# yixuan/ADMM

Measured on AMD Instinct MI355X. Metric: ADMM iterations/sec, Lasso tall n=100000 p=10000 (100-lambda warm-started path), higher is better.
Workload: dtype f32; 1 GPU; admm_lasso tall path (BASELINE configs[1]); n=100000, p=10000, nlambda=100, standardize=True, intercept=True, parallelism=single GPU, step=one cold-started warm-chained lambda path

## Files before the change

### admm_amd/csrc/symv_kernels.h

```cpp
#pragma once
#include "admm_internal.h"
#include "device_utils.h"
#include "symv_pack.h"
#include <hip/hip_ext.h>
#include <climits>
#include <type_traits>

namespace admm {

constexpr int kSyRB = 256;
constexpr int kSyCB = 128;
constexpr int kSyCBMax = 256;
static_assert(kSyCBMax == 256, "SYMV_SCHED's widths are checked against 256 where the option is parsed (options.hip)");
constexpr int kSyThreads = 256;

struct SymvSched {
    int width_big = kSyCB, width_small = kSyCB;
    int rb_split = 0;
    __host__ __device__ int width(int rb) const { return rb >= rb_split ? width_big : width_small; }
    __host__ __device__ int nseg(int rb, int p32) const {
        const int cols = min((rb + 1) * kSyRB, p32), w = width(rb);
        return (cols + w - 1) / w;
    }
};
constexpr int kSySumLanes = 8;

struct SymvArgs {
    const float* A; long long lda; int p;
    const float* v0; const float* v1;
    float* dot0; float* dot1;
    float* axp0; float* axp1;
    long long ldo;
    const int4* tiles;
    const int* skip;
    const unsigned long long* verdict;
    unsigned long long discard;
    unsigned long long* early;
#ifdef ADMM_HIP_PROBE
    long long* probe; int probe_idx;
#endif
};

constexpr int kSyVerdictReplicas = 64;
constexpr int kSyVerdictStride = 16;
struct SymvVerdict {
    const unsigned long long* words = nullptr;
    unsigned long long discard = 0;
    unsigned long long* early = nullptr;
    bool mid = false;
};

template <typename T>
__device__ __forceinline__ T butterfly8(const T (&v)[8], int lane) {
    T a4[4], a2[2];
    {
        const int b = (lane >> 5) & 1;
#pragma unroll
        for (int k = 0; k < 4; ++k) {
            const T keep = b ? v[k + 4] : v[k], send = b ? v[k] : v[k + 4];
            a4[k] = keep + __shfl_xor(send, 32, 64);
        }
    }
    {
        const int b = (lane >> 4) & 1;
#pragma unroll
        for (int k = 0; k < 2; ++k) {
            const T keep = b ? a4[k + 2] : a4[k], send = b ? a4[k] : a4[k + 2];
            a2[k] = keep + __shfl_xor(send, 16, 64);
        }
    }
    const int b = (lane >> 3) & 1;
    const T keep = b ? a2[1] : a2[0], send = b ? a2[0] : a2[1];
    T r = keep + __shfl_xor(send, 8, 64);
    r += __shfl_xor(r, 4, 64);
    r += __shfl_xor(r, 2, 64);
    r += __shfl_xor(r, 1, 64);
    return r;
}

struct SymvPlainVec {
    __device__ __forceinline__ float4 load4(const float* p) const { return *reinterpret_cast<const float4*>(p); }
    __device__ __forceinline__ float load1(const float* p) const { return *p; }
};
struct SymvBypassVec {
    __device__ __forceinline__ float4 load4(const float* p) const {
        const unsigned long long lo = __hip_atomic_load(reinterpret_cast<const unsigned long long*>(p), __ATOMIC_RELAXED, __HIP_MEMORY_SCOPE_AGENT);
        const unsigned long long hi = __hip_atomic_load(reinterpret_cast<const unsigned long long*>(p) + 1, __ATOMIC_RELAXED, __HIP_MEMORY_SCOPE_AGENT);
        return make_float4(__uint_as_float((unsigned)lo), __uint_as_float((unsigned)(lo >> 32)), __uint_as_float((unsigned)hi), __uint_as_float((unsigned)(hi >> 32)));
    }
    __device__ __forceinline__ float load1(const float* p) const {
        return __uint_as_float(__hip_atomic_load(reinterpret_cast<const unsigned int*>(p), __ATOMIC_RELAXED, __HIP_MEMORY_SCOPE_AGENT));
    }
};
struct SymvNoWait { __device__ __forceinline__ void operator()() const {} };

template <bool PRE, typename Wait, typename VecLoad, bool NT = false, bool MID = false>
__device__ __forceinline__ void symv2_tile(const SymvArgs& a, const int4 t, Wait wait, VecLoad vl,
                                           float4 (*red)[kSyThreads], float (*sdot)[kSyCBMax]) {
    const int rb = t.x, seg = t.w;
    const int cw = t.z >> 2;
    const int lane = threadIdx.x & 63, wid = threadIdx.x >> 6;
    const int row = rb * kSyRB + lane * 4;
    const int col0 = t.y + wid * cw;
    const int p4 = (a.p + 3) & ~3;
    const bool active = row < p4;
    const bool has = col0 < a.p;
    const float* base = a.A + (size_t)col0 * a.lda + row;
    float4 av[8];
    if (PRE) {
#pragma unroll
        for (int k = 0; k < 8; ++k) {
            av[k] = make_float4(0.f, 0.f, 0.f, 0.f);
            if (has && active && col0 + k < a.p) av[k] = *reinterpret_cast<const float4*>(base + (size_t)k * a.lda);
        }
        wait();
    }
    float4 aU = make_float4(0.f, 0.f, 0.f, 0.f), aW = aU;

    if (has) {
        const float4 uI = active ? vl.load4(a.v0 + row) : make_float4(0.f, 0.f, 0.f, 0.f);
        const float4 wI = active ? vl.load4(a.v1 + row) : make_float4(0.f, 0.f, 0.f, 0.f);
        const int cj = col0 + lane;
        const float uj = (lane < cw && cj < a.p) ? vl.load1(a.v0 + cj) : 0.f;
        const float wj = (lane < cw && cj < a.p) ? vl.load1(a.v1 + cj) : 0.f;
        const bool diag = col0 + (cw - 1) >= rb * kSyRB;
        const int nq = cw >> 3;
        const int last = active ? min(a.p - 1, diag ? row + 3 : INT_MAX) : -1;
        const unsigned long long* vword = a.verdict + (size_t)(blockIdx.x & (kSyVerdictReplicas - 1)) * kSyVerdictStride;
#pragma unroll 1
        for (int q = 0; q < nq; ++q) {
            unsigned long long vq = 0;
            if constexpr (MID) vq = __hip_atomic_load(vword, __ATOMIC_RELAXED, __HIP_MEMORY_SCOPE_AGENT);
            if (!PRE || q > 0) {
#pragma unroll
                for (int k = 0; k < 8; ++k) {
                    const int col = col0 + q * 8 + k;
                    av[k] = make_float4(0.f, 0.f, 0.f, 0.f);
                    if constexpr (NT) { if (col <= last) av[k] = load16_nt<float4>(base + (size_t)(q * 8 + k) * a.lda); }
                    else { if (col <= last) av[k] = *reinterpret_cast<const float4*>(base + (size_t)(q * 8 + k) * a.lda); }
                }
            }
            if constexpr (MID) {
                const unsigned lo = __builtin_amdgcn_readfirstlane((unsigned)vq), hi = __builtin_amdgcn_readfirstlane((unsigned)(vq >> 32));
                if ((((unsigned long long)hi << 32) | lo) == a.discard) break;
            }
            float dU[8], dW[8];
#pragma unroll
            for (int k = 0; k < 8; ++k) {
                const int col = col0 + q * 8 + k;
                float4 v = av[k];
                float4 ax = v;
                if (diag) {
                    if (row + 0 < col) v.x = 0.f;
                    if (row + 1 < col) v.y = 0.f;
                    if (row + 2 < col) v.z = 0.f;
                    if (row + 3 < col) v.w = 0.f;
                    ax = v;
                    if (row + 0 == col) ax.x = 0.f;
                    if (row + 1 == col) ax.y = 0.f;
                    if (row + 2 == col) ax.z = 0.f;
                    if (row + 3 == col) ax.w = 0.f;
                }
                dU[k] = fmaf(v.x, uI.x, fmaf(v.y, uI.y, fmaf(v.z, uI.z, v.w * uI.w)));
                dW[k] = fmaf(v.x, wI.x, fmaf(v.y, wI.y, fmaf(v.z, wI.z, v.w * wI.w)));
                const float ujc = __int_as_float(__builtin_amdgcn_readlane(__float_as_int(uj), (q * 8 + k) & 63));
                const float wjc = __int_as_float(__builtin_amdgcn_readlane(__float_as_int(wj), (q * 8 + k) & 63));
                aU.x = fmaf(ax.x, ujc, aU.x); aU.y = fmaf(ax.y, ujc, aU.y); aU.z = fmaf(ax.z, ujc, aU.z); aU.w = fmaf(ax.w, ujc, aU.w);
                aW.x = fmaf(ax.x, wjc, aW.x); aW.y = fmaf(ax.y, wjc, aW.y); aW.z = fmaf(ax.z, wjc, aW.z); aW.w = fmaf(ax.w, wjc, aW.w);
            }
            const float du = butterfly8(dU, lane);
            const float dw = butterfly8(dW, lane);
            if ((lane & 7) == 0) {
                sdot[0][wid * cw + q * 8 + (lane >> 3)] = du;
                sdot[1][wid * cw + q * 8 + (lane >> 3)] = dw;
            }
        }
    } else {
        for (int c = lane; c < cw; c += 64) { sdot[0][wid * cw + c] = 0.f; sdot[1][wid * cw + c] = 0.f; }
    }
    red[0][threadIdx.x] = aU;
    red[1][threadIdx.x] = aW;
    __syncthreads();
    if (wid < 2) {
        float4 s = red[wid][lane];
#pragma unroll
        for (int ww = 1; ww < 4; ++ww) {
            const float4 o = red[wid][ww * 64 + lane];
            s.x += o.x; s.y += o.y; s.z += o.z; s.w += o.w;
        }
        float* dst = (wid == 0 ? a.axp0 : a.axp1) + (size_t)seg * a.ldo + row;
        *reinterpret_cast<float4*>(dst) = s;
    } else {
        float* dst = (wid == 2 ? a.dot0 : a.dot1) + (size_t)rb * a.ldo + t.y;
        for (int c = lane * 4; c < t.z; c += 256) *reinterpret_cast<float4*>(dst + c) = *reinterpret_cast<const float4*>(&sdot[wid - 2][c]);
    }
}

struct SymvNoExtra { __device__ void operator()() const {} };

template <typename Extra, bool NT = false, bool MID = false>
__global__ void __launch_bounds__(kSyThreads, 4)
symv2_lower_kernel(SymvArgs a, Extra extra) {
    if (blockIdx.x == 0) { extra(); return; }
    const int4 t = a.tiles[blockIdx.x - 1];
    const unsigned long long vw = __hip_atomic_load(a.verdict + (size_t)(blockIdx.x & (kSyVerdictReplicas - 1)) * kSyVerdictStride,
                                                    __ATOMIC_RELAXED, __HIP_MEMORY_SCOPE_AGENT);
    const int done = *a.skip;
    if (done != 0) return;
    if (vw == a.discard) {
        if (threadIdx.x == 0) atomicAdd(a.early, 1ull);
        return;
    }
    __shared__ float4 red[2][kSyThreads];
    __shared__ __attribute__((aligned(16))) float sdot[2][kSyCBMax];
#ifdef ADMM_HIP_PROBE
    const long long pt0 = wall_clock64();
#endif
    symv2_tile<false, SymvNoWait, SymvPlainVec, NT, MID>(a, t, SymvNoWait(), SymvPlainVec(), red, sdot);
#ifdef ADMM_HIP_PROBE
    if (a.probe != nullptr && threadIdx.x == 0) {
        const int nt = (int)gridDim.x - 1, t = (int)blockIdx.x - 1;
        const int which = t == 0 ? 0 : (t == nt / 2 ? 1 : (t == nt - 1 ? 2 : (t == (3 * nt) / 4 ? 3 : -1)));
        if (which >= 0) {
            long long* d = a.probe + ((size_t)(a.probe_idx & 4095) * 4 + 3) * 8 + which * 2;
            d[0] = pt0; d[1] = wall_clock64();
        }
    }
#endif
}

constexpr int kSyGateLeave = -1;
constexpr int kSyEarlySlots = kSyVerdictReplicas;
constexpr int kSyGateScratch = 6 * (kSyThreads / 64);
struct SymvForcedGate {
    struct Req {};
    int answer;
    __device__ __forceinline__ Req request() const { return Req(); }
    __device__ __forceinline__ int decide(const Req&, double*) const { return answer; }
};
#ifndef ADMM_HIP_SYMV1_WGS
#define ADMM_HIP_SYMV1_WGS 4
#endif
#ifndef ADMM_HIP_SYMV1_PRE
#define ADMM_HIP_SYMV1_PRE 8
#endif

struct SymvTileGeom { int row, col0, last, lane, wid, nqw; };

struct SymvDenseSrc {
    struct Desc {};
    __device__ __forceinline__ Desc describe(int) const { return Desc(); }
    template <bool NT>
    struct Chunk {
        const float* base; long long lda; int col0, last;
        float4 av[8];
        __device__ __forceinline__ Chunk(const SymvDenseSrc&, const Desc&, const SymvArgs& a, const SymvTileGeom& g)
            : base(a.A + (size_t)g.col0 * a.lda + g.row), lda(a.lda), col0(g.col0), last(g.last) {}
        template <int K0, int K1>
        __device__ __forceinline__ void request(int q) {
#pragma unroll
            for (int k = K0; k < K1; ++k) {
                const int col = col0 + q * 8 + k;
                av[k] = make_float4(0.f, 0.f, 0.f, 0.f);
                if constexpr (NT) { if (col <= last) av[k] = load16_nt<float4>(base + (size_t)(q * 8 + k) * lda); }
                else { if (col <= last) av[k] = *reinterpret_cast<const float4*>(base + (size_t)(q * 8 + k) * lda); }
            }
        }
        __device__ __forceinline__ void get(int, float4 (&out)[8]) const {
#pragma unroll
            for (int k = 0; k < 8; ++k) out[k] = av[k];
        }
    };
};

struct SymvPackedSrc {
    const unsigned* stream;
    const int4* ptile;
    const uint2* esc;
    int esc_cap;
    using Desc = int4;
    __device__ __forceinline__ Desc describe(int tile) const { return ptile[tile]; }
    template <bool NT>
    struct Chunk {
        const unsigned* mine;
        const uint2* esc; int nesc, ebase, col0, last, lane, chunk0;
        uint4 pc[kSpPieces]; unsigned signs;
        __device__ __forceinline__ Chunk(const SymvPackedSrc& s, const Desc& d, const SymvArgs&, const SymvTileGeom& g)
            : mine(s.stream + ((size_t)d.x + (size_t)(g.wid * g.nqw)) * kSpChunkDwords + g.lane * 4), esc(s.esc + (size_t)(blockIdx.x - 1) * s.esc_cap),
              nesc(d.z), ebase(d.y), col0(g.col0), last(g.last), lane(g.lane), chunk0(g.wid * g.nqw) {}
        template <int K0, int K1>
        __device__ __forceinline__ void request(int q) {
            if constexpr (K0 == 0 && K1 > 0) {
                const unsigned* c = mine + (size_t)q * kSpChunkDwords;
                pc[0] = make_uint4(0xEEEEEEEEu, 0xEEEEEEEEu, 0xEEEEEEEEu, 0xEEEEEEEEu);
#pragma unroll
                for (int i = 1; i < kSpPieces; ++i) pc[i] = make_uint4(0u, 0u, 0u, 0u);
                signs = 0u;
                if (col0 + q * 8 <= last) {
                    if constexpr (NT) {
#pragma unroll
                        for (int i = 0; i < kSpPieces; ++i) pc[i] = load16_nt<uint4>(c + i * 256);
                        signs = __builtin_nontemporal_load(c + 4 * kSpPieces * 64 - 3 * lane);
                    } else {
#pragma unroll
                        for (int i = 0; i < kSpPieces; ++i) pc[i] = *reinterpret_cast<const uint4*>(c + i * 256);
                        signs = c[4 * kSpPieces * 64 - 3 * lane];
                    }
                }
            }
        }
        __device__ __forceinline__ void get(int q, float4 (&out)[8]) const {
            unsigned rec[kSpRecDwords], bits[kSpEntries];
#pragma unroll
            for (int i = 0; i < kSpPieces; ++i) { rec[4 * i] = pc[i].x; rec[4 * i + 1] = pc[i].y; rec[4 * i + 2] = pc[i].z; rec[4 * i + 3] = pc[i].w; }
            rec[4 * kSpPieces] = signs;
#if ADMM_HIP_SYMV_PACK_DEC == 2
#pragma unroll
            for (int e = 0; e < kSpEntries; ++e) bits[e] = rec[e < kSpRecDwords ? e : e - 4] ^ (unsigned)ebase;
#else
            sp_record_decode(rec, ebase, bits);
#endif
#pragma unroll
            for (int k = 0; k < 8; ++k)
                out[k] = make_float4(__uint_as_float(bits[4 * k]), __uint_as_float(bits[4 * k + 1]), __uint_as_float(bits[4 * k + 2]), __uint_as_float(bits[4 * k + 3]));
            if (nesc > 0) {
                const unsigned me = ((unsigned)(chunk0 + q) << 6) | (unsigned)lane;
                for (int i = 0; i < nesc; ++i) {
                    const uint2 en = esc[i];
                    const bool hit = (en.x >> 5) == me;
                    const unsigned e = en.x & 31u;
                    const float val = __uint_as_float(en.y);
#pragma unroll
                    for (int k = 0; k < 8; ++k) {
                        if (hit && e == 4u * k + 0u) out[k].x = val;
                        if (hit && e == 4u * k + 1u) out[k].y = val;
                        if (hit && e == 4u * k + 2u) out[k].z = val;
                        if (hit && e == 4u * k + 3u) out[k].w = val;
                    }
                }
            }
        }
    };
};

template <typename Src, typename Gate, bool NT, int PRE>
__device__ __forceinline__ void symv1_tile(const SymvArgs& a, const Src& src, const Gate& gate, float4* red, float* sdot, double* gate_lds) {
    const int4 t = a.tiles[blockIdx.x - 1];
    const int done = *a.skip;
    const typename Gate::Req greq = gate.request();
    const typename Src::Desc sd = src.describe(blockIdx.x - 1);
    if (done != 0) return;
    const int rb = t.x, seg = t.w;
    const int cw = t.z >> 2;
    const int lane = threadIdx.x & 63, wid = threadIdx.x >> 6;
    const int row = rb * kSyRB + lane * 4;
    const int col0 = t.y + wid * cw;
    const int p4 = (a.p + 3) & ~3;
    const bool active = row < p4;
    const bool has = col0 < a.p;
    const bool diag = col0 + (cw - 1) >= rb * kSyRB;
    const int nq = has ? cw >> 3 : 0;
    const int last = active ? min(a.p - 1, diag ? row + 3 : INT_MAX) : -1;
    const SymvTileGeom geom = {row, col0, last, lane, wid, cw >> 3};
    typename Src::template Chunk<NT> ch(src, sd, a, geom);
    static_assert(PRE >= 0 && PRE <= 8, "columns of the first chunk requested ahead of the gate");
    if constexpr (PRE > 0) { if (nq > 0) ch.template request<0, PRE>(0); }
    const int g = gate.decide(greq, gate_lds);
    if (g == kSyGateLeave) {
        if (threadIdx.x == 0) atomicAdd(a.early + (size_t)(blockIdx.x & (kSyEarlySlots - 1)) * kSyVerdictStride, 1ull);
        return;
    }
#ifdef ADMM_HIP_PROBE
    const long long pt0 = wall_clock64();
#endif
    const float* v = g != 0 ? a.v1 : a.v0;
    float4 aU = make_float4(0.f, 0.f, 0.f, 0.f);
    if (has) {
        const float4 uI = active ? *reinterpret_cast<const float4*>(v + row) : make_float4(0.f, 0.f, 0.f, 0.f);
        const int cj = col0 + lane;
        const float uj = (lane < cw && cj < a.p) ? v[cj] : 0.f;
        const auto consume = [&](int q) {
            float4 av[8];
            ch.get(q, av);
            float dU[8];
#pragma unroll
            for (int k = 0; k < 8; ++k) {
                const int col = col0 + q * 8 + k;
                float4 m = av[k];
                float4 ax = m;
                if (diag) {
                    if (row + 0 < col) m.x = 0.f;
                    if (row + 1 < col) m.y = 0.f;
                    if (row + 2 < col) m.z = 0.f;
                    if (row + 3 < col) m.w = 0.f;
                    ax = m;
                    if (row + 0 == col) ax.x = 0.f;
                    if (row + 1 == col) ax.y = 0.f;
                    if (row + 2 == col) ax.z = 0.f;
                    if (row + 3 == col) ax.w = 0.f;
                }
                dU[k] = fmaf(m.x, uI.x, fmaf(m.y, uI.y, fmaf(m.z, uI.z, m.w * uI.w)));
                const float ujc = __int_as_float(__builtin_amdgcn_readlane(__float_as_int(uj), (q * 8 + k) & 63));
                aU.x = fmaf(ax.x, ujc, aU.x); aU.y = fmaf(ax.y, ujc, aU.y); aU.z = fmaf(ax.z, ujc, aU.z); aU.w = fmaf(ax.w, ujc, aU.w);
            }
            const float du = butterfly8(dU, lane);
            if ((lane & 7) == 0) sdot[wid * cw + q * 8 + (lane >> 3)] = du;
        };
        if constexpr (PRE > 0) { ch.template request<PRE, 8>(0); consume(0); }
#pragma unroll 1
        for (int q = PRE > 0 ? 1 : 0; q < nq; ++q) {
            ch.template request<0, 8>(q);
            consume(q);
        }
    } else {
        for (int c = lane; c < cw; c += 64) sdot[wid * cw + c] = 0.f;
    }
    red[threadIdx.x] = aU;
    __syncthreads();
    if (wid == 0) {
        float4 s = red[lane];
#pragma unroll
        for (int ww = 1; ww < 4; ++ww) {
            const float4 o = red[ww * 64 + lane];
            s.x += o.x; s.y += o.y; s.z += o.z; s.w += o.w;
        }
        *reinterpret_cast<float4*>(a.axp0 + (size_t)seg * a.ldo + row) = s;
    } else if (wid == 1) {
        float* dst = a.dot0 + (size_t)rb * a.ldo + t.y;
        for (int c = lane * 4; c < t.z; c += 256) *reinterpret_cast<float4*>(dst + c) = *reinterpret_cast<const float4*>(&sdot[c]);
    }
#ifdef ADMM_HIP_PROBE
    if (a.probe != nullptr && threadIdx.x == 0) {
        const int nt = (int)gridDim.x - 1, ti = (int)blockIdx.x - 1;
        const int which = ti == 0 ? 0 : (ti == nt / 2 ? 1 : (ti == nt - 1 ? 2 : (ti == (3 * nt) / 4 ? 3 : -1)));
        if (which >= 0) {
            long long* d = a.probe + ((size_t)(a.probe_idx & 4095) * 4 + 3) * 8 + which * 2;
            d[0] = pt0; d[1] = wall_clock64();
        }
    }
#endif
}

template <typename Gate, typename Extra, bool NT = false, int PRE = ADMM_HIP_SYMV1_PRE>
__global__ void __launch_bounds__(kSyThreads, ADMM_HIP_SYMV1_WGS)
symv1_lower_kernel(SymvArgs a, Gate gate, Extra extra) {
    if (blockIdx.x == 0) { extra(); return; }
    __shared__ float4 red[kSyThreads];
    __shared__ __attribute__((aligned(16))) float sdot[kSyCBMax];
    __shared__ double gate_lds[kSyGateScratch];
    symv1_tile<SymvDenseSrc, Gate, NT, PRE>(a, SymvDenseSrc(), gate, red, sdot, gate_lds);
}

template <typename Gate, typename Extra, bool NT = false, int PRE = ADMM_HIP_SYMV1_PRE>
__global__ void __launch_bounds__(kSyThreads, ADMM_HIP_SYMV1_WGS)
symv1_packed_kernel(SymvArgs a, SymvPackedSrc src, Gate gate, Extra extra) {
    if (blockIdx.x == 0) { extra(); return; }
    __shared__ float4 red[kSyThreads];
    __shared__ __attribute__((aligned(16))) float sdot[kSyCBMax];
    __shared__ double gate_lds[kSyGateScratch];
    symv1_tile<SymvPackedSrc, Gate, NT, PRE>(a, src, gate, red, sdot, gate_lds);
}

struct SymvPackArgs {
    const float* A; long long lda; int p;
    const int4* tiles;
    int4* ptile;
    unsigned* stream;
    uint2* esc; int esc_cap;
    unsigned long long* totals;
};
static __global__ void __launch_bounds__(kSyThreads)
symv_pack_kernel(SymvPackArgs a) {
    __shared__ int s_base;
    __shared__ unsigned s_cnt;
    const int4 t = a.tiles[blockIdx.x];
    const int rb = t.x, cw = t.z >> 2, nqw = cw >> 3;
    const int lane = threadIdx.x & 63, wid = threadIdx.x >> 6;
    const int row = rb * kSyRB + lane * 4;
    const int col0 = t.y + wid * cw;
    const int p4 = (a.p + 3) & ~3;
    const bool active = row < p4;
    if (threadIdx.x == 0) { s_base = 0; s_cnt = 0u; }
    __syncthreads();
    const float* base = a.A + (size_t)col0 * a.lda + row;
    const auto column = [&](int j, unsigned (&b)[4]) {
        const int col = col0 + j;
        b[0] = b[1] = b[2] = b[3] = 0u;
        if (active && col < a.p && row + 3 >= col) {
            const float4 m = *reinterpret_cast<const float4*>(base + (size_t)j * a.lda);
            if (row + 0 >= col) b[0] = __float_as_uint(m.x);
            if (row + 1 >= col) b[1] = __float_as_uint(m.y);
            if (row + 2 >= col) b[2] = __float_as_uint(m.z);
            b[3] = __float_as_uint(m.w);
        }
    };
    int mx = 0;
    for (int j = 0; j < cw; ++j) {
        unsigned b[4];
        column(j, b);
#pragma unroll
        for (int c = 0; c < 4; ++c) if (sp_counts(b[c])) mx = max(mx, sp_exp7(b[c]));
    }
    atomicMax(&s_base, mx);
    __syncthreads();
    const int ebase = s_base;
    const size_t first = (size_t)a.ptile[blockIdx.x].x;
    for (int q = 0; q < nqw; ++q) {
        unsigned bits[kSpEntries], rec[kSpRecDwords];
#pragma unroll
        for (int k = 0; k < 8; ++k) {
            unsigned b[4];
            column(q * 8 + k, b);
            bits[4 * k] = b[0]; bits[4 * k + 1] = b[1]; bits[4 * k + 2] = b[2]; bits[4 * k + 3] = b[3];
        }
        const unsigned em = sp_record_encode(bits, ebase, rec);
        unsigned* c = a.stream + (first + (size_t)(wid * nqw + q)) * kSpChunkDwords;
#pragma unroll
        for (int i = 0; i < kSpPieces; ++i)
            *reinterpret_cast<uint4*>(c + (i * 64 + lane) * 4) = make_uint4(rec[4 * i], rec[4 * i + 1], rec[4 * i + 2], rec[4 * i + 3]);
        c[4 * kSpPieces * 64 + lane] = rec[4 * kSpPieces];
        if (em != 0u) {
#pragma unroll
            for (int e = 0; e < kSpEntries; ++e) {
                if ((em >> e) & 1u) {
                    const unsigned slot = atomicAdd(&s_cnt, 1u);
                    if (slot < (unsigned)a.esc_cap)
                        a.esc[(size_t)blockIdx.x * a.esc_cap + slot] = make_uint2(((unsigned)(wid * nqw + q) << 11) | ((unsigned)lane << 5) | (unsigned)e, bits[e]);
                }
            }
        }
    }
    __syncthreads();
    if (threadIdx.x == 0) {
        const unsigned n = s_cnt;
        int4 d = a.ptile[blockIdx.x];
        d.y = ebase; d.z = (int)min(n, (unsigned)a.esc_cap); d.w = (int)n;
        a.ptile[blockIdx.x] = d;
        if (n != 0u) atomicAdd(a.totals, (unsigned long long)n);
        if (n > (unsigned)a.esc_cap) atomicAdd(a.totals + 1, 1ull);
    }
}

struct SymvNArgs {
    const float* A; long long lda; int p;
    const float* v; long long vstride;
    float* dot; long long dot_stride;
    float* axp; long long axp_stride;
    int nvec;
    long long ldo;
    const int4* tiles;
    const int* skip;
};
constexpr int kSyNR[] = {2, 4, 8, 12};
constexpr int kSyNRCount = (int)(sizeof(kSyNR) / sizeof(kSyNR[0]));

template <int NR, bool DIAG>
__device__ __forceinline__ void symvn_chunk(float4 (&av)[8], const float4 (&vI)[NR], const float (&vj)[NR], float4 (&acc)[NR],
                                            int row, int colq, int q, int lane, float (*sdot)[kSyCBMax], int sbase) {
    float4 ax[DIAG ? 8 : 1];
    if (DIAG) {
#pragma unroll
        for (int k = 0; k < 8; ++k) {
            const int col = colq + k;
            float4 v = av[k];
            if (row + 0 < col) v.x = 0.f;
            if (row + 1 < col) v.y = 0.f;
            if (row + 2 < col) v.z = 0.f;
            if (row + 3 < col) v.w = 0.f;
            av[k] = v;
            if (row + 0 == col) v.x = 0.f;
            if (row + 1 == col) v.y = 0.f;
            if (row + 2 == col) v.z = 0.f;
            if (row + 3 == col) v.w = 0.f;
            ax[DIAG ? k : 0] = v;
        }
    }
#pragma unroll
    for (int r = 0; r < NR; ++r) {
        float d[8];
        const float4 xi = vI[r];
        float4 s = acc[r];
#pragma unroll
        for (int k = 0; k < 8; ++k) {
            const float4 v = av[k];
            const float4 x = DIAG ? ax[DIAG ? k : 0] : av[k];
            d[k] = fmaf(v.x, xi.x, fmaf(v.y, xi.y, fmaf(v.z, xi.z, v.w * xi.w)));
            const float c = __int_as_float(__builtin_amdgcn_readlane(__float_as_int(vj[r]), (q * 8 + k) & 63));
            s.x = fmaf(x.x, c, s.x); s.y = fmaf(x.y, c, s.y); s.z = fmaf(x.z, c, s.z); s.w = fmaf(x.w, c, s.w);
        }
        acc[r] = s;
        const float dr = butterfly8(d, lane);
        if ((lane & 7) == 0) sdot[r][sbase + (lane >> 3)] = dr;
    }
}

template <int NR, typename Extra, bool NT = false>
__global__ void __launch_bounds__(kSyThreads, 2)
symvn_lower_kernel(SymvNArgs a, Extra extra) {
    static_assert(NR >= 2 && NR % 2 == 0, "right-hand sides come in pairs (u_k, w_k)");
    if (blockIdx.x == 0) { extra(); return; }
    if (a.skip != nullptr && *a.skip != 0) return;
    __shared__ float4 red[2][kSyThreads];
    __shared__ __attribute__((aligned(16))) float sdot[NR][kSyCBMax];
    const int4 t = a.tiles[blockIdx.x - 1];
    const int rb = t.x, seg = t.w;
    const int cw = t.z >> 2;
    const int lane = threadIdx.x & 63, wid = threadIdx.x >> 6;
    const int row = rb * kSyRB + lane * 4;
    const int col0 = t.y + wid * cw;
    const int p4 = (a.p + 3) & ~3;
    const bool active = row < p4;
    const bool has = col0 < a.p;
    const float* base = a.A + (size_t)col0 * a.lda + row;
    float4 acc[NR];
#pragma unroll
    for (int r = 0; r < NR; ++r) acc[r] = make_float4(0.f, 0.f, 0.f, 0.f);

    if (has) {
        float4 vI[NR];
        float vj[NR];
        const int cj = col0 + lane;
#pragma unroll
        for (int r = 0; r < NR; ++r) {
            const float* vr = a.v + (size_t)min(r, a.nvec - 1) * a.vstride;
            vI[r] = active ? *reinterpret_cast<const float4*>(vr + row) : make_float4(0.f, 0.f, 0.f, 0.f);
            vj[r] = (lane < cw && cj < a.p) ? vr[cj] : 0.f;
        }
        const bool diag = col0 + (cw - 1) >= rb * kSyRB;
        const int nq = cw >> 3;
#pragma unroll 1
        for (int q = 0; q < nq; ++q) {
            float4 av[8];
#pragma unroll
            for (int k = 0; k < 8; ++k) {
                const int col = col0 + q * 8 + k;
                av[k] = make_float4(0.f, 0.f, 0.f, 0.f);
                if constexpr (NT) { if (active && col < a.p) av[k] = load16_nt<float4>(base + (size_t)(q * 8 + k) * a.lda); }
                else { if (active && col < a.p) av[k] = *reinterpret_cast<const float4*>(base + (size_t)(q * 8 + k) * a.lda); }
            }
            if (diag) symvn_chunk<NR, true>(av, vI, vj, acc, row, col0 + q * 8, q, lane, sdot, wid * cw + q * 8);
            else symvn_chunk<NR, false>(av, vI, vj, acc, row, col0 + q * 8, q, lane, sdot, wid * cw + q * 8);
        }
    } else {
#pragma unroll
        for (int r = 0; r < NR; ++r)
            for (int c = lane; c < cw; c += 64) sdot[r][wid * cw + c] = 0.f;
    }
#pragma unroll
    for (int pr = 0; pr < NR / 2; ++pr) {
        if (pr > 0) __syncthreads();
        red[0][threadIdx.x] = acc[2 * pr];
        red[1][threadIdx.x] = acc[2 * pr + 1];
        __syncthreads();
        const int r = 2 * pr + (wid & 1);
        if (r >= a.nvec) continue;
        if (wid < 2) {
            float4 s = red[wid][lane];
#pragma unroll
            for (int ww = 1; ww < 4; ++ww) {
                const float4 o = red[wid][ww * 64 + lane];
                s.x += o.x; s.y += o.y; s.z += o.z; s.w += o.w;
            }
            float* dst = a.axp + (size_t)r * a.axp_stride + (size_t)seg * a.ldo + row;
            *reinterpret_cast<float4*>(dst) = s;
        } else {
            float* dst = a.dot + (size_t)r * a.dot_stride + (size_t)rb * a.ldo + t.y;
            for (int c = lane * 4; c < t.z; c += 256) *reinterpret_cast<float4*>(dst + c) = *reinterpret_cast<const float4*>(&sdot[r][c]);
        }
    }
}

struct SymvArgsD {
    const float* A; long long lda; int p;
    const float* v0; const float* v1;
    double* dot0; double* dot1; double* axp0; double* axp1;
    long long ldo;
    const int4* tiles;
    const int* skip;
};
static __global__ void __launch_bounds__(kSyThreads, 2)
symv2_lower_f64acc_kernel(SymvArgsD a) {
    if (a.skip != nullptr && *a.skip != 0) return;
    __shared__ double4 red[2][kSyThreads];
    __shared__ __attribute__((aligned(16))) double sdot[2][kSyCBMax];
    const int4 t = a.tiles[blockIdx.x];
    const int rb = t.x, seg = t.w, cw = t.z >> 2;
    const int lane = threadIdx.x & 63, wid = threadIdx.x >> 6;
    const int row = rb * kSyRB + lane * 4;
    const int col0 = t.y + wid * cw;
    const int p4 = (a.p + 3) & ~3;
    const bool active = row < p4, has = col0 < a.p;
    const float* base = a.A + (size_t)col0 * a.lda + row;
    double4 aU = make_double4(0, 0, 0, 0), aW = aU;
    if (has) {
        const float4 uI = active ? *reinterpret_cast<const float4*>(a.v0 + row) : make_float4(0.f, 0.f, 0.f, 0.f);
        const float4 wI = active ? *reinterpret_cast<const float4*>(a.v1 + row) : make_float4(0.f, 0.f, 0.f, 0.f);
        const int cj = col0 + lane;
        const float uj = (lane < cw && cj < a.p) ? a.v0[cj] : 0.f;
        const float wj = (lane < cw && cj < a.p) ? a.v1[cj] : 0.f;
        const bool diag = col0 + (cw - 1) >= rb * kSyRB;
        for (int q = 0; q < (cw >> 3); ++q) {
            double dU[8], dW[8];
#pragma unroll
            for (int k = 0; k < 8; ++k) {
                const int col = col0 + q * 8 + k;
                float4 v = make_float4(0.f, 0.f, 0.f, 0.f);
                if (active && col < a.p) v = *reinterpret_cast<const float4*>(base + (size_t)(q * 8 + k) * a.lda);
                float4 ax = v;
                if (diag) {
                    if (row + 0 < col) v.x = 0.f;
                    if (row + 1 < col) v.y = 0.f;
                    if (row + 2 < col) v.z = 0.f;
                    if (row + 3 < col) v.w = 0.f;
                    ax = v;
                    if (row + 0 == col) ax.x = 0.f;
                    if (row + 1 == col) ax.y = 0.f;
                    if (row + 2 == col) ax.z = 0.f;
                    if (row + 3 == col) ax.w = 0.f;
                }
                dU[k] = (double)v.x * uI.x + (double)v.y * uI.y + (double)v.z * uI.z + (double)v.w * uI.w;
                dW[k] = (double)v.x * wI.x + (double)v.y * wI.y + (double)v.z * wI.z + (double)v.w * wI.w;
                const double ujc = (double)__int_as_float(__builtin_amdgcn_readlane(__float_as_int(uj), (q * 8 + k) & 63));
                const double wjc = (double)__int_as_float(__builtin_amdgcn_readlane(__float_as_int(wj), (q * 8 + k) & 63));
                aU.x += ax.x * ujc; aU.y += ax.y * ujc; aU.z += ax.z * ujc; aU.w += ax.w * ujc;
                aW.x += ax.x * wjc; aW.y += ax.y * wjc; aW.z += ax.z * wjc; aW.w += ax.w * wjc;
            }
            const double du = butterfly8(dU, lane), dw = butterfly8(dW, lane);
            if ((lane & 7) == 0) { sdot[0][wid * cw + q * 8 + (lane >> 3)] = du; sdot[1][wid * cw + q * 8 + (lane >> 3)] = dw; }
        }
    } else {
        for (int c = lane; c < cw; c += 64) { sdot[0][wid * cw + c] = 0.0; sdot[1][wid * cw + c] = 0.0; }
    }
    red[0][threadIdx.x] = aU;
    red[1][threadIdx.x] = aW;
    __syncthreads();
    if (wid < 2) {
        double4 s = red[wid][lane];
#pragma unroll
        for (int ww = 1; ww < 4; ++ww) { const double4 o = red[wid][ww * 64 + lane]; s.x += o.x; s.y += o.y; s.z += o.z; s.w += o.w; }
        double* dst = (wid == 0 ? a.axp0 : a.axp1) + (size_t)seg * a.ldo + row;
        dst[0] = s.x; dst[1] = s.y; dst[2] = s.z; dst[3] = s.w;
    } else {
        double* dst = (wid == 2 ? a.dot0 : a.dot1) + (size_t)rb * a.ldo + t.y;
        for (int c = lane; c < t.z; c += 64) dst[c] = sdot[wid - 2][c];
    }
}

struct SymvLayout {
    int p = 0, nrb = 0, ncb = 0, p32 = 0;
    int nax_rows = 0;
    SymvSched sched;
    long long ldo = 0;
    bool nt = false;
    std::vector<int4> tiles;
};

inline SymvLayout symv_plan_layout(int p, int cus, int part, int nparts) {
    SymvLayout L;
    const int p32 = (p + 31) / 32 * 32;
    const int nrb = (p + kSyRB - 1) / kSyRB;
    L.p = p; L.p32 = p32; L.nrb = nrb;
    L.ncb = (p + kSyCB - 1) / kSyCB;
    L.ldo = (long long)nrb * kSyRB;
    SymvSched sched;
    auto count = [&](const SymvSched& sc) { long long t = 0; for (int rb = 0; rb < nrb; ++rb) t += sc.nseg(rb, p32); return t; };
    const long long slots = 4ll * cus * std::max(1, nparts);
    auto uniform = [](int w) { SymvSched sc; sc.width_big = sc.width_small = w; sc.rb_split = 0; return sc; };
    auto two = [&](int wb, int ws) { SymvSched sc; sc.width_big = wb; sc.width_small = ws; sc.rb_split = nrb / 2; return sc; };
    if (4 * count(uniform(32)) <= 3 * slots) sched = uniform(32);
    else if (count(uniform(64)) <= slots) sched = uniform(64);
    else if (10 * count(two(128, 64)) <= 14 * slots) sched = two(128, 64);
    else sched = two(192, 64);
    if (const OptValue* v = opt(Opt::SYMV_SCHED)) {
        sched.width_big = v->sched[0]; sched.width_small = v->sched[1]; sched.rb_split = (int)((long long)v->sched[2] * nrb / 1000);
    }
    std::vector<int4> h;
    int nax_rows = 1;
    for (int rb = nrb - 1; rb >= 0; --rb) {
        const int w = sched.width(rb), ns = sched.nseg(rb, p32);
        nax_rows = std::max(nax_rows, ns);
        for (int sg = 0; sg < ns; ++sg) {
            const int c0 = sg * w;
            const int cols = std::min((rb + 1) * kSyRB, p32);
            h.push_back(make_int4(rb, c0, std::min(w, cols - c0), sg));
        }
    }
    if (nparts > 1) {
        auto gcd = [](int a, int b) { while (b) { const int t = a % b; a = b; b = t; } return a; };
        std::vector<int4> mine;
        int group = -1, last_rb = -1, last_cg = -1;
        for (const int4& t : h) {
            const int w = sched.width(t.x);
            const int gw = w / gcd(w, 128) * 128;
            const int cg = t.y / gw;
            if (t.x != last_rb || cg != last_cg) { ++group; last_rb = t.x; last_cg = cg; }
            if (group % nparts == part) mine.push_back(t);
        }
        h.swap(mine);
    }
    L.nt = (size_t)2 * (size_t)p * (size_t)p / (size_t)std::max(1, nparts) > (size_t)310000000;
    L.sched = sched; L.nax_rows = nax_rows;
    L.tiles.swap(h);
    return L;
}

struct SymvPlan {
    int p = 0, nrb = 0, ncb = 0, ntiles = 0, p32 = 0;
    int nax_rows = 0;
    SymvSched sched;
    long long ldo = 0;
    DevBuf<int4> tiles;
    std::vector<int4> htiles;
    bool nt = false;
    DevBuf<float> dot0, dot1, axp0, axp1;
    DevBuf<unsigned long long> zero;
#ifdef ADMM_HIP_PROBE
    long long* probe = nullptr; mutable int probe_idx = 0;
#endif
    void init(int p_, hipStream_t st, int part = 0, int nparts = 1) {
        int cus = 256;
        { int dev = 0; hipDeviceProp_t prop; if (hipGetDevice(&dev) == hipSuccess && hipGetDeviceProperties(&prop, dev) == hipSuccess) cus = prop.multiProcessorCount; }
        SymvLayout L = symv_plan_layout(p_, cus, part, nparts);
        p = L.p; nrb = L.nrb; ncb = L.ncb; p32 = L.p32; nax_rows = L.nax_rows; sched = L.sched; ldo = L.ldo; nt = L.nt;
        htiles.swap(L.tiles);
        const std::vector<int4>& h = htiles;
        ntiles = (int)h.size();
        tiles.alloc(std::max<size_t>(h.size(), 1));
        if (!h.empty()) ADMM_HIP_CHECK(hipMemcpyAsync(tiles.get(), h.data(), h.size() * sizeof(int4), hipMemcpyHostToDevice, st));
        dot0.alloc((size_t)nrb * ldo); dot1.alloc((size_t)nrb * ldo);
        axp0.alloc((size_t)nax_rows * ldo); axp1.alloc((size_t)nax_rows * ldo);
        dot0.zero(st); dot1.zero(st); axp0.zero(st); axp1.zero(st);
        zero.alloc((size_t)kSyVerdictReplicas * kSyVerdictStride); zero.zero(st);
        ADMM_HIP_CHECK(hipStreamSynchronize(st));
    }
    SymvArgs args(const float* A, long long lda, const float* v0, const float* v1, const int* skip, const SymvVerdict& vd = SymvVerdict()) const {
        SymvArgs a;
        a.A = A; a.lda = lda; a.p = p; a.v0 = v0; a.v1 = v1;
        a.dot0 = dot0.get(); a.dot1 = dot1.get(); a.axp0 = axp0.get(); a.axp1 = axp1.get();
        a.ldo = ldo; a.tiles = tiles.get();
        a.skip = skip != nullptr ? skip : reinterpret_cast<const int*>(zero.get());
        a.verdict = vd.words != nullptr ? vd.words : zero.get();
        a.discard = vd.words != nullptr ? vd.discard : ~0ull;
        a.early = vd.early;
#ifdef ADMM_HIP_PROBE
        a.probe = probe; a.probe_idx = probe_idx++;
#endif
        return a;
    }
    template <typename Extra = SymvNoExtra>
    void launch(const float* A, long long lda, const float* v0, const float* v1, const int* skip, hipStream_t st, Extra extra = Extra(),
                hipEvent_t ev_start = nullptr, hipEvent_t ev_stop = nullptr, const SymvVerdict& vd = SymvVerdict()) {
        const SymvArgs a = args(A, lda, v0, v1, skip, vd);
        if (nt) {
            if (ev_start == nullptr && ev_stop == nullptr) hipLaunchKernelGGL((symv2_lower_kernel<Extra, true>), dim3(ntiles + 1), dim3(kSyThreads), 0, st, a, extra);
            else hipExtLaunchKernelGGL((symv2_lower_kernel<Extra, true>), dim3(ntiles + 1), dim3(kSyThreads), 0, st, ev_start, ev_stop, 0, a, extra);
            return;
        }
        if (vd.words != nullptr && vd.mid) {
            if (ev_start == nullptr && ev_stop == nullptr) hipLaunchKernelGGL((symv2_lower_kernel<Extra, false, true>), dim3(ntiles + 1), dim3(kSyThreads), 0, st, a, extra);
            else hipExtLaunchKernelGGL((symv2_lower_kernel<Extra, false, true>), dim3(ntiles + 1), dim3(kSyThreads), 0, st, ev_start, ev_stop, 0, a, extra);
            return;
        }
        if (ev_start == nullptr && ev_stop == nullptr) hipLaunchKernelGGL((symv2_lower_kernel<Extra>), dim3(ntiles + 1), dim3(kSyThreads), 0, st, a, extra);
        else hipExtLaunchKernelGGL((symv2_lower_kernel<Extra>), dim3(ntiles + 1), dim3(kSyThreads), 0, st, ev_start, ev_stop, 0, a, extra);
    }
    template <typename Gate, typename Extra = SymvNoExtra>
    void launch_one(const float* A, long long lda, const float* v0, const float* v1, const int* skip, hipStream_t st, Gate gate, unsigned long long* early,
                    Extra extra = Extra(), hipEvent_t ev_start = nullptr, hipEvent_t ev_stop = nullptr) {
        SymvVerdict vd;
        vd.early = early;
        const SymvArgs a = args(A, lda, v0, v1, skip, vd);
        const bool timed = ev_start != nullptr || ev_stop != nullptr;
        if (nt) {
            if (!timed) hipLaunchKernelGGL((symv1_lower_kernel<Gate, Extra, true>), dim3(ntiles + 1), dim3(kSyThreads), 0, st, a, gate, extra);
            else hipExtLaunchKernelGGL((symv1_lower_kernel<Gate, Extra, true>), dim3(ntiles + 1), dim3(kSyThreads), 0, st, ev_start, ev_stop, 0, a, gate, extra);
            return;
        }
        if (!timed) hipLaunchKernelGGL((symv1_lower_kernel<Gate, Extra>), dim3(ntiles + 1), dim3(kSyThreads), 0, st, a, gate, extra);
        else hipExtLaunchKernelGGL((symv1_lower_kernel<Gate, Extra>), dim3(ntiles + 1), dim3(kSyThreads), 0, st, ev_start, ev_stop, 0, a, gate, extra);
    }
};

struct SymvPacked {
    DevBuf<unsigned> stream;
    DevBuf<int4> ptile;
    DevBuf<uint2> esc;
    DevBuf<unsigned long long> totals;
    int esc_cap = kSpEscCap;
    size_t chunks = 0;
    unsigned long long escapes = 0, overflowed = 0;
    bool ready = false, nt = false;
    size_t bytes() const { return chunks * (size_t)kSpChunkBytes; }
    static size_t bytes_for(const SymvPlan& sy) {
        size_t c = 0;
        for (const int4& t : sy.htiles) c += (size_t)(t.z >> 3);
        return c * (size_t)kSpChunkBytes;
    }
    void release() { stream.release(); ptile.release(); esc.release(); totals.release(); chunks = 0; ready = false; }
    bool build(const SymvPlan& sy, const float* A, long long lda, hipStream_t st, int cap = kSpEscCap) {
        ready = false;
        esc_cap = cap;
        std::vector<int4> h((size_t)std::max(sy.ntiles, 1), make_int4(0, 0, 0, 0));
        chunks = 0;
        for (int k = 0; k < sy.ntiles; ++k) { h[k].x = (int)chunks; chunks += (size_t)(sy.htiles[k].z >> 3); }
        if (sy.ntiles == 0) return false;
        stream.alloc(chunks * (size_t)kSpChunkDwords);
        ptile.alloc(h.size());
        esc.alloc(std::max<size_t>((size_t)sy.ntiles * (size_t)cap, 1));
        totals.alloc(2); totals.zero(st);
        ADMM_HIP_CHECK(hipMemcpyAsync(ptile.get(), h.data(), h.size() * sizeof(int4), hipMemcpyHostToDevice, st));
        SymvPackArgs a;
        a.A = A; a.lda = lda; a.p = sy.p; a.tiles = sy.tiles.get(); a.ptile = ptile.get(); a.stream = stream.get();
        a.esc = esc.get(); a.esc_cap = cap; a.totals = totals.get();
        hipLaunchKernelGGL(symv_pack_kernel, dim3(sy.ntiles), dim3(kSyThreads), 0, st, a);
        ADMM_HIP_CHECK(hipGetLastError());
        unsigned long long tt[2] = {0, 0};
        ADMM_HIP_CHECK(hipMemcpyAsync(tt, totals.get(), sizeof(tt), hipMemcpyDeviceToHost, st));
        ADMM_HIP_CHECK(hipStreamSynchronize(st));
        escapes = tt[0]; overflowed = tt[1];
        nt = bytes() > (size_t)310000000;
        ready = overflowed == 0;
        return ready;
    }
    SymvPackedSrc src() const { return SymvPackedSrc{stream.get(), ptile.get(), esc.get(), esc_cap}; }
};

template <typename Gate, typename Extra = SymvNoExtra>
void symv_launch_one_packed(const SymvPlan& sy, const SymvPacked& pk, const float* v0, const float* v1, const int* skip, hipStream_t st, Gate gate,
                            unsigned long long* early, Extra extra = Extra(), hipEvent_t ev_start = nullptr, hipEvent_t ev_stop = nullptr) {
    SymvVerdict vd;
    vd.early = early;
    const SymvArgs a = sy.args(nullptr, 0, v0, v1, skip, vd);
    const SymvPackedSrc src = pk.src();
    const bool timed = ev_start != nullptr || ev_stop != nullptr;
    if (pk.nt) {
        if (!timed) hipLaunchKernelGGL((symv1_packed_kernel<Gate, Extra, true>), dim3(sy.ntiles + 1), dim3(kSyThreads), 0, st, a, src, gate, extra);
        else hipExtLaunchKernelGGL((symv1_packed_kernel<Gate, Extra, true>), dim3(sy.ntiles + 1), dim3(kSyThreads), 0, st, ev_start, ev_stop, 0, a, src, gate, extra);
        return;
    }
    if (!timed) hipLaunchKernelGGL((symv1_packed_kernel<Gate, Extra>), dim3(sy.ntiles + 1), dim3(kSyThreads), 0, st, a, src, gate, extra);
    else hipExtLaunchKernelGGL((symv1_packed_kernel<Gate, Extra>), dim3(sy.ntiles + 1), dim3(kSyThreads), 0, st, ev_start, ev_stop, 0, a, src, gate, extra);
}

template <int NL, typename T = float>
__device__ __forceinline__ void symv_sum_partials(const T* __restrict__ dot0, const T* __restrict__ dot1,
                                                  const T* __restrict__ axp0, const T* __restrict__ axp1,
                                                  long long ldo, int nrb, const SymvSched sched, int p32, int i, int sub, bool valid, T& a, T& b) {
    const int ic = valid ? i : 0;
    const int rbi = ic / kSyRB;
    const int rb0 = rbi;
    const int ndot = nrb - rb0;
    const int nax = sched.nseg(rbi, p32);
    const int ntot = valid ? ndot + nax : 0;
    const unsigned ld = (unsigned)ldo;
    a = T(0); b = T(0);
    for (int k0 = 0; k0 < ntot; k0 += 16 * NL) {
        T va[16], vb[16];
#pragma unroll
        for (int j = 0; j < 16; ++j) {
            const int k = k0 + j * NL + sub;
            const bool isdot = k < ndot;
            const int row = isdot ? rb0 + k : min(k, ntot - 1) - ndot;
            const unsigned o = (unsigned)row * ld + (unsigned)ic;
            va[j] = (isdot ? dot0 : axp0)[o];
            vb[j] = (isdot ? dot1 : axp1)[o];
        }
        __builtin_amdgcn_sched_barrier(0);
#pragma unroll
        for (int j = 0; j < 16; ++j) {
            const bool in = k0 + j * NL + sub < ntot;
            a += in ? va[j] : T(0); b += in ? vb[j] : T(0);
        }
    }
#pragma unroll
    for (int m = 1; m < NL; m <<= 1) { a += __shfl_xor(a, m, 64); b += __shfl_xor(b, m, 64); }
}

template <int NL, typename T = float>
__device__ __forceinline__ T symv_sum_partials1(const T* __restrict__ dot0, const T* __restrict__ axp0,
                                                long long ldo, int nrb, const SymvSched sched, int p32, int i, int sub, bool valid) {
    const int ic = valid ? i : 0;
    const int rbi = ic / kSyRB;
    const int rb0 = rbi;
    const int ndot = nrb - rb0;
    const int nax = sched.nseg(rbi, p32);
    const int ntot = valid ? ndot + nax : 0;
    const unsigned ld = (unsigned)ldo;
    T a = T(0);
    for (int k0 = 0; k0 < ntot; k0 += 16 * NL) {
        T va[16];
#pragma unroll
        for (int j = 0; j < 16; ++j) {
            const int k = k0 + j * NL + sub;
            const bool isdot = k < ndot;
            const int row = isdot ? rb0 + k : min(k, ntot - 1) - ndot;
            const unsigned o = (unsigned)row * ld + (unsigned)ic;
            va[j] = (isdot ? dot0 : axp0)[o];
        }
        __builtin_amdgcn_sched_barrier(0);
#pragma unroll
        for (int j = 0; j < 16; ++j) {
            const bool in = k0 + j * NL + sub < ntot;
            a += in ? va[j] : T(0);
        }
    }
#pragma unroll
    for (int m = 1; m < NL; m <<= 1) a += __shfl_xor(a, m, 64);
    return a;
}

template <typename Extra>
void symvn_launch(const SymvPlan& sy, int nr, const SymvNArgs& a, hipStream_t st, Extra extra, hipEvent_t ev_start = nullptr, hipEvent_t ev_stop = nullptr) {
    const dim3 grid(sy.ntiles + 1), block(kSyThreads);
    const bool timed = ev_start != nullptr || ev_stop != nullptr;
#define ADMM_SYMVN_LAUNCH(NR, NT)                                                                                                        \
    if (timed) hipExtLaunchKernelGGL((symvn_lower_kernel<NR, Extra, NT>), grid, block, 0, st, ev_start, ev_stop, 0, a, extra);           \
    else hipLaunchKernelGGL((symvn_lower_kernel<NR, Extra, NT>), grid, block, 0, st, a, extra)
#define ADMM_SYMVN_CASE(NR)                                                                                                              \
    case NR:                                                                                                                             \
        if (sy.nt) { ADMM_SYMVN_LAUNCH(NR, true); } else { ADMM_SYMVN_LAUNCH(NR, false); }                                               \
        break;
    switch (nr) {
        ADMM_SYMVN_CASE(2) ADMM_SYMVN_CASE(4) ADMM_SYMVN_CASE(8) ADMM_SYMVN_CASE(12)
        default: throw Error(ADMM_ERR_INTERNAL, "symvn_lower_kernel is not built for that many right-hand sides per pass");
    }
#undef ADMM_SYMVN_CASE
#undef ADMM_SYMVN_LAUNCH
}

constexpr int kMtChunk = 4;
template <int NL, int KB>
__device__ __forceinline__ void symv_sum_partials_n(const float* __restrict__ dot, long long dot_stride, const float* __restrict__ axp, long long axp_stride,
                                                    int npair, long long ldo, int nrb, const SymvSched sched, int p32, int i, int sub, bool valid,
                                                    float (&a)[KB], float (&b)[KB]) {
    const int ic = valid ? i : 0;
    const int rbi = ic / kSyRB;
    const int ndot = nrb - rbi;
    const int nax = sched.nseg(rbi, p32);
    const int ntot = valid ? ndot + nax : 0;
    const unsigned ld = (unsigned)ldo;
#pragma unroll
    for (int k = 0; k < KB; ++k) { a[k] = 0.f; b[k] = 0.f; }
    for (int k0 = 0; k0 < ntot; k0 += 8 * NL) {
        float va[KB][8], vb[KB][8];
#pragma unroll
        for (int k = 0; k < KB; ++k) {
            const int kc = min(k, npair - 1);
            const float* d0 = dot + (size_t)(2 * kc) * dot_stride; const float* d1 = d0 + dot_stride;
            const float* x0 = axp + (size_t)(2 * kc) * axp_stride; const float* x1 = x0 + axp_stride;
#pragma unroll
            for (int j = 0; j < 8; ++j) {
                const int s = k0 + j * NL + sub;
                const bool isdot = s < ndot;
                const int row = isdot ? rbi + s : min(s, ntot - 1) - ndot;
                const unsigned o = (unsigned)row * ld + (unsigned)ic;
                va[k][j] = (isdot ? d0 : x0)[o];
                vb[k][j] = (isdot ? d1 : x1)[o];
            }
        }
        __builtin_amdgcn_sched_barrier(0);
#pragma unroll
        for (int k = 0; k < KB; ++k) {
#pragma unroll
            for (int j = 0; j < 8; ++j) {
                const bool in = k0 + j * NL + sub < ntot && k < npair;
                a[k] += in ? va[k][j] : 0.f; b[k] += in ? vb[k][j] : 0.f;
            }
        }
    }
#pragma unroll
    for (int k = 0; k < KB; ++k) {
#pragma unroll
        for (int m = 1; m < NL; m <<= 1) { a[k] += __shfl_xor(a[k], m, 64); b[k] += __shfl_xor(b[k], m, 64); }
    }
}

}
```

Before: 27300 iterations/s.

## Double-buffer packed SYMV chunk loads via buffer resources in ping-pong registers

```diff
diff --git a/admm_amd/csrc/symv_kernels.h b/admm_amd/csrc/symv_kernels.h
--- a/admm_amd/csrc/symv_kernels.h
+++ b/admm_amd/csrc/symv_kernels.h
@@ -82,20 +82,9 @@
     __device__ __forceinline__ float4 load4(const float* p) const { return *reinterpret_cast<const float4*>(p); }
     __device__ __forceinline__ float load1(const float* p) const { return *p; }
 };
-struct SymvBypassVec {
-    __device__ __forceinline__ float4 load4(const float* p) const {
-        const unsigned long long lo = __hip_atomic_load(reinterpret_cast<const unsigned long long*>(p), __ATOMIC_RELAXED, __HIP_MEMORY_SCOPE_AGENT);
-        const unsigned long long hi = __hip_atomic_load(reinterpret_cast<const unsigned long long*>(p) + 1, __ATOMIC_RELAXED, __HIP_MEMORY_SCOPE_AGENT);
-        return make_float4(__uint_as_float((unsigned)lo), __uint_as_float((unsigned)(lo >> 32)), __uint_as_float((unsigned)hi), __uint_as_float((unsigned)(hi >> 32)));
-    }
-    __device__ __forceinline__ float load1(const float* p) const {
-        return __uint_as_float(__hip_atomic_load(reinterpret_cast<const unsigned int*>(p), __ATOMIC_RELAXED, __HIP_MEMORY_SCOPE_AGENT));
-    }
-};
-struct SymvNoWait { __device__ __forceinline__ void operator()() const {} };
-
-template <bool PRE, typename Wait, typename VecLoad, bool NT = false, bool MID = false>
-__device__ __forceinline__ void symv2_tile(const SymvArgs& a, const int4 t, Wait wait, VecLoad vl,
+
+template <typename VecLoad, bool NT = false, bool MID = false>
+__device__ __forceinline__ void symv2_tile(const SymvArgs& a, const int4 t, VecLoad vl,
                                            float4 (*red)[kSyThreads], float (*sdot)[kSyCBMax]) {
     const int rb = t.x, seg = t.w;
     const int cw = t.z >> 2;
@@ -107,14 +96,6 @@
     const bool has = col0 < a.p;
     const float* base = a.A + (size_t)col0 * a.lda + row;
     float4 av[8];
-    if (PRE) {
-#pragma unroll
-        for (int k = 0; k < 8; ++k) {
-            av[k] = make_float4(0.f, 0.f, 0.f, 0.f);
-            if (has && active && col0 + k < a.p) av[k] = *reinterpret_cast<const float4*>(base + (size_t)k * a.lda);
-        }
-        wait();
-    }
     float4 aU = make_float4(0.f, 0.f, 0.f, 0.f), aW = aU;
 
     if (has) {
@@ -131,14 +112,12 @@
         for (int q = 0; q < nq; ++q) {
             unsigned long long vq = 0;
             if constexpr (MID) vq = __hip_atomic_load(vword, __ATOMIC_RELAXED, __HIP_MEMORY_SCOPE_AGENT);
-            if (!PRE || q > 0) {
-#pragma unroll
-                for (int k = 0; k < 8; ++k) {
-                    const int col = col0 + q * 8 + k;
-                    av[k] = make_float4(0.f, 0.f, 0.f, 0.f);
-                    if constexpr (NT) { if (col <= last) av[k] = load16_nt<float4>(base + (size_t)(q * 8 + k) * a.lda); }
-                    else { if (col <= last) av[k] = *reinterpret_cast<const float4*>(base + (size_t)(q * 8 + k) * a.lda); }
-                }
+#pragma unroll
+            for (int k = 0; k < 8; ++k) {
+                const int col = col0 + q * 8 + k;
+                av[k] = make_float4(0.f, 0.f, 0.f, 0.f);
+                if constexpr (NT) { if (col <= last) av[k] = load16_nt<float4>(base + (size_t)(q * 8 + k) * a.lda); }
+                else { if (col <= last) av[k] = *reinterpret_cast<const float4*>(base + (size_t)(q * 8 + k) * a.lda); }
             }
             if constexpr (MID) {
                 const unsigned lo = __builtin_amdgcn_readfirstlane((unsigned)vq), hi = __builtin_amdgcn_readfirstlane((unsigned)(vq >> 32));
@@ -216,7 +195,7 @@
 #ifdef ADMM_HIP_PROBE
     const long long pt0 = wall_clock64();
 #endif
-    symv2_tile<false, SymvNoWait, SymvPlainVec, NT, MID>(a, t, SymvNoWait(), SymvPlainVec(), red, sdot);
+    symv2_tile<SymvPlainVec, NT, MID>(a, t, SymvPlainVec(), red, sdot);
 #ifdef ADMM_HIP_PROBE
     if (a.probe != nullptr && threadIdx.x == 0) {
         const int nt = (int)gridDim.x - 1, t = (int)blockIdx.x - 1;
@@ -241,6 +220,9 @@
 #ifndef ADMM_HIP_SYMV1_WGS
 #define ADMM_HIP_SYMV1_WGS 4
 #endif
+#ifndef ADMM_HIP_SYMV1_DEPTH
+#define ADMM_HIP_SYMV1_DEPTH 2
+#endif
 #ifndef ADMM_HIP_SYMV1_PRE
 #define ADMM_HIP_SYMV1_PRE 8
 #endif
@@ -248,6 +230,8 @@
 struct SymvTileGeom { int row, col0, last, lane, wid, nqw; };
 
 struct SymvDenseSrc {
+    static constexpr int kDepth = 1;
+    static __device__ __forceinline__ int wave_id() { return threadIdx.x >> 6; }
     struct Desc {};
     __device__ __forceinline__ Desc describe(int) const { return Desc(); }
     template <bool NT>
@@ -266,6 +250,7 @@
                 else { if (col <= last) av[k] = *reinterpret_cast<const float4*>(base + (size_t)(q * 8 + k) * lda); }
             }
         }
+        template <int B = 0>
         __device__ __forceinline__ void get(int, float4 (&out)[8]) const {
 #pragma unroll
             for (int k = 0; k < 8; ++k) out[k] = av[k];
@@ -280,40 +265,51 @@
     int esc_cap;
     using Desc = int4;
     __device__ __forceinline__ Desc describe(int tile) const { return ptile[tile]; }
+    static constexpr int kDepth = ADMM_HIP_SYMV1_DEPTH;
+    static __device__ __forceinline__ int wave_id() { return __builtin_amdgcn_readfirstlane(threadIdx.x >> 6); }
+    static constexpr unsigned kNoRequest = 0x7FFF0000u;
+    struct Rec { uint4 pc[kSpPieces]; unsigned signs; };
     template <bool NT>
     struct Chunk {
-        const unsigned* mine;
+        __amdgpu_buffer_rsrc_t chunks;
+        unsigned off16, off4;
         const uint2* esc; int nesc, ebase, col0, last, lane, chunk0;
-        uint4 pc[kSpPieces]; unsigned signs;
+        Rec ping, pong;
         __device__ __forceinline__ Chunk(const SymvPackedSrc& s, const Desc& d, const SymvArgs&, const SymvTileGeom& g)
-            : mine(s.stream + ((size_t)d.x + (size_t)(g.wid * g.nqw)) * kSpChunkDwords + g.lane * 4), esc(s.esc + (size_t)(blockIdx.x - 1) * s.esc_cap),
-              nesc(d.z), ebase(d.y), col0(g.col0), last(g.last), lane(g.lane), chunk0(g.wid * g.nqw) {}
-        template <int K0, int K1>
-        __device__ __forceinline__ void request(int q) {
+            : off16(g.lane * 16u), off4((4u * kSpPieces * 64u + g.lane) * 4u), esc(s.esc + (size_t)(blockIdx.x - 1) * s.esc_cap),
+              nesc(d.z), ebase(d.y), col0(g.col0), last(g.last), lane(g.lane), chunk0(g.wid * g.nqw) {
+            const int w = g.wid, first = __builtin_amdgcn_readfirstlane(d.x), nqw = __builtin_amdgcn_readfirstlane(g.nqw);
+            const unsigned* base = s.stream + ((size_t)first + (size_t)(w * nqw)) * kSpChunkDwords;
+            chunks = __builtin_amdgcn_make_buffer_rsrc(const_cast<unsigned*>(base), 0, nqw * kSpChunkBytes, 0x00020000);
+        }
+        template <int B> __device__ __forceinline__ Rec& rec() { if constexpr (B == 0) return ping; else return pong; }
+        template <int B> __device__ __forceinline__ const Rec& rec() const { if constexpr (B == 0) return ping; else return pong; }
+        __device__ __forceinline__ bool requested(int q) const { return col0 + q * 8 <= last; }
+        template <int K0, int K1, int B = 0>
+        __device__ __forceinline__ void request(int q, bool exists = true) {
             if constexpr (K0 == 0 && K1 > 0) {
-                const unsigned* c = mine + (size_t)q * kSpChunkDwords;
-                pc[0] = make_uint4(0xEEEEEEEEu, 0xEEEEEEEEu, 0xEEEEEEEEu, 0xEEEEEEEEu);
-#pragma unroll
-                for (int i = 1; i < kSpPieces; ++i) pc[i] = make_uint4(0u, 0u, 0u, 0u);
-                signs = 0u;
-                if (col0 + q * 8 <= last) {
-                    if constexpr (NT) {
-#pragma unroll
-                        for (int i = 0; i < kSpPieces; ++i) pc[i] = load16_nt<uint4>(c + i * 256);
-                        signs = __builtin_nontemporal_load(c + 4 * kSpPieces * 64 - 3 * lane);
-                    } else {
-#pragma unroll
-                        for (int i = 0; i < kSpPieces; ++i) pc[i] = *reinterpret_cast<const uint4*>(c + i * 256);
-                        signs = c[4 * kSpPieces * 64 - 3 * lane];
-                    }
+                typedef unsigned int u4_t __attribute__((ext_vector_type(4)));
+                constexpr int aux = NT ? 2 : 0;
+                Rec& r = rec<B>();
+                const bool on = exists && requested(q);
+                const unsigned at = (unsigned)q * (unsigned)kSpChunkBytes;
+                const unsigned o16 = on ? at + off16 : kNoRequest, o4 = on ? at + off4 : kNoRequest;
+#pragma unroll
+                for (int i = 0; i < kSpPieces; ++i) {
+                    const u4_t v = __builtin_amdgcn_raw_buffer_load_b128(chunks, o16 + 1024u * i, 0, aux);
+                    r.pc[i] = make_uint4(v.x, v.y, v.z, v.w);
                 }
-            }
-        }
+                r.signs = __builtin_amdgcn_raw_buffer_load_b32(chunks, o4, 0, aux);
+            }
+        }
+        template <int B = 0>
         __device__ __forceinline__ void get(int q, float4 (&out)[8]) const {
+            const Rec& r = rec<B>();
             unsigned rec[kSpRecDwords], bits[kSpEntries];
 #pragma unroll
-            for (int i = 0; i < kSpPieces; ++i) { rec[4 * i] = pc[i].x; rec[4 * i + 1] = pc[i].y; rec[4 * i + 2] = pc[i].z; rec[4 * i + 3] = pc[i].w; }
-            rec[4 * kSpPieces] = signs;
+            for (int i = 0; i < kSpPieces; ++i) { rec[4 * i] = r.pc[i].x; rec[4 * i + 1] = r.pc[i].y; rec[4 * i + 2] = r.pc[i].z; rec[4 * i + 3] = r.pc[i].w; }
+            rec[4 * kSpPieces] = r.signs;
+            if (!requested(q)) { rec[0] = 0xEEEEEEEEu; rec[1] = 0xEEEEEEEEu; rec[2] = 0xEEEEEEEEu; rec[3] = 0xEEEEEEEEu; }
 #if ADMM_HIP_SYMV_PACK_DEC == 2
 #pragma unroll
             for (int e = 0; e < kSpEntries; ++e) bits[e] = rec[e < kSpRecDwords ? e : e - 4] ^ (unsigned)ebase;
@@ -352,7 +348,7 @@
     if (done != 0) return;
     const int rb = t.x, seg = t.w;
     const int cw = t.z >> 2;
-    const int lane = threadIdx.x & 63, wid = threadIdx.x >> 6;
+    const int lane = threadIdx.x & 63, wid = Src::wave_id();
     const int row = rb * kSyRB + lane * 4;
     const int col0 = t.y + wid * cw;
     const int p4 = (a.p + 3) & ~3;
@@ -379,9 +375,9 @@
         const float4 uI = active ? *reinterpret_cast<const float4*>(v + row) : make_float4(0.f, 0.f, 0.f, 0.f);
         const int cj = col0 + lane;
         const float uj = (lane < cw && cj < a.p) ? v[cj] : 0.f;
-        const auto consume = [&](int q) {
+        const auto consume = [&](int q, auto buf) {
             float4 av[8];
-            ch.get(q, av);
+            ch.template get<decltype(buf)::value>(q, av);
             float dU[8];
 #pragma unroll
             for (int k = 0; k < 8; ++k) {
@@ -406,11 +402,29 @@
             const float du = butterfly8(dU, lane);
             if ((lane & 7) == 0) sdot[wid * cw + q * 8 + (lane >> 3)] = du;
         };
-        if constexpr (PRE > 0) { ch.template request<PRE, 8>(0); consume(0); }
+        constexpr std::integral_constant<int, 0> ping;
+        constexpr std::integral_constant<int, 1> pong;
+        if constexpr (Src::kDepth == 2) {
+            if constexpr (PRE > 0) ch.template request<PRE, 8, 0>(0); else ch.template request<0, 8, 0>(0);
 #pragma unroll 1
-        for (int q = PRE > 0 ? 1 : 0; q < nq; ++q) {
-            ch.template request<0, 8>(q);
-            consume(q);
+            for (int q = 0; q < nq; q += 2) {
+                __builtin_amdgcn_sched_barrier(0);
+                ch.template request<0, 8, 1>(q + 1, q + 1 < nq);
+                __builtin_amdgcn_sched_barrier(0);
+                consume(q, ping);
+                if (q + 1 >= nq) break;
+                __builtin_amdgcn_sched_barrier(0);
+                ch.template request<0, 8, 0>(q + 2, q + 2 < nq);
+                __builtin_amdgcn_sched_barrier(0);
+                consume(q + 1, pong);
+            }
+        } else {
+            if constexpr (PRE > 0) { ch.template request<PRE, 8>(0); consume(0, ping); }
+#pragma unroll 1
+            for (int q = PRE > 0 ? 1 : 0; q < nq; ++q) {
+                ch.template request<0, 8>(q);
+                consume(q, ping);
+            }
         }
     } else {
         for (int c = lane; c < cw; c += 64) sdot[wid * cw + c] = 0.f;
```

Result: faster. 27780 iterations/s, median of 6 (+1.8%).
